# ZechengLi19/CIM

Measured on NVIDIA B200. Metric: CIM-head images/s (ROIAlign fwd+bwd + mask IoU + scoring fwd+bwd + mining + losses incl. PCL), higher is better.
Workload: dtype f32

## Files before the change

cim_b200/csrc/common.cuh:

```cuda
#pragma once
#include <cuda_runtime.h>
#include <cuda_fp16.h>
#include <stdint.h>
#include "../../include/cimhead.h"

#if defined(__CUDA_ARCH__) && (__CUDA_ARCH__ < 1000)
#error "libcimhead is written for sm_100a (B200) only"
#endif

#define CIM_API extern "C" __attribute__((visibility("default")))

static inline int cim_launch_status() {
    cudaError_t e = cudaGetLastError();
    return e == cudaSuccess ? CIM_OK : (int)e;
}
static inline bool cim_aligned(const void *p, size_t a) { return ((uintptr_t)p % a) == 0; }
static inline int cim_num_sms() {
    int dev = 0, n = 148;
    if (cudaGetDevice(&dev) == cudaSuccess)
        cudaDeviceGetAttribute(&n, cudaDevAttrMultiProcessorCount, dev);
    return n > 0 ? n : 148;
}
static inline int cim_max_smem_optin() {
    int dev = 0, n = 0;
    if (cudaGetDevice(&dev) == cudaSuccess)
        cudaDeviceGetAttribute(&n, cudaDevAttrMaxSharedMemoryPerBlockOptin, dev);
    return n;
}

__device__ __forceinline__ uint32_t smem_u32(const void *p) {
    return (uint32_t)__cvta_generic_to_shared(p);
}
__device__ __forceinline__ void mbar_init(uint64_t *bar, uint32_t count) {
    asm volatile("mbarrier.init.shared::cta.b64 [%0], %1;" ::"r"(smem_u32(bar)), "r"(count));
}
__device__ __forceinline__ void mbar_expect_tx(uint64_t *bar, uint32_t bytes) {
    asm volatile("mbarrier.arrive.expect_tx.shared::cta.b64 _, [%0], %1;" ::"r"(smem_u32(bar)),
                 "r"(bytes)
                 : "memory");
}
__device__ __forceinline__ void mbar_wait(uint64_t *bar, uint32_t parity) {
    asm volatile(
        "{\n\t.reg .pred p;\n\t"
        "WAIT_%=:\n\t"
        "mbarrier.try_wait.parity.shared::cta.b64 p, [%0], %1, %2;\n\t"
        "@p bra DONE_%=;\n\t"
        "bra WAIT_%=;\n\t"
        "DONE_%=:\n\t}" ::"r"(smem_u32(bar)),
        "r"(parity), "r"(100000u)
        : "memory");
}
__device__ __forceinline__ bool elect_one() {
    uint32_t leader;
    asm volatile("{\n\t.reg .pred p;\n\telect.sync _|p, 0xffffffff;\n\tselp.u32 %0, 1, 0, p;\n\t}" : "=r"(leader));
    return leader != 0;
}
__device__ __forceinline__ void fence_mbar_init() {
    asm volatile("fence.mbarrier_init.release.cluster;" ::: "memory");
}
__device__ __forceinline__ void fence_proxy_async_smem() {
    asm volatile("fence.proxy.async.shared::cta;" ::: "memory");
}
__device__ __forceinline__ void bulk_g2s(void *smem_dst, const void *gmem_src, uint32_t bytes,
                                         uint64_t *bar) {
    asm volatile(
        "cp.async.bulk.shared::cluster.global.mbarrier::complete_tx::bytes [%0], [%1], %2, [%3];" ::
            "r"(smem_u32(smem_dst)),
        "l"(gmem_src), "r"(bytes), "r"(smem_u32(bar))
        : "memory");
}
__device__ __forceinline__ void bulk_s2g(void *gmem_dst, const void *smem_src, uint32_t bytes) {
    asm volatile("cp.async.bulk.global.shared::cta.bulk_group [%0], [%1], %2;" ::"l"(gmem_dst),
                 "r"(smem_u32(smem_src)), "r"(bytes)
                 : "memory");
}
__device__ __forceinline__ void bulk_commit() { asm volatile("cp.async.bulk.commit_group;" ::: "memory"); }
template <int N>
__device__ __forceinline__ void bulk_wait_read() {
    asm volatile("cp.async.bulk.wait_group.read %0;" ::"n"(N) : "memory");
}
template <int N>
__device__ __forceinline__ void bulk_wait() {
    asm volatile("cp.async.bulk.wait_group %0;" ::"n"(N) : "memory");
}
```

cim_b200/csrc/mask_overlap.cu:

```cuda
#include "common.cuh"

bool cim_mask_overlap_tc_eligible(int n, long long words);
int cim_mask_overlap_tc_launch(const uint32_t *packed, const int32_t *area, const int32_t *perm,
                               const uint32_t *umap_a, const uint32_t *umap_b, int bw, unsigned long long *visited,
                               const int32_t *tile_order, int n_img, int n, long long words, int32_t *inter,
                               __half *iou, __half *asy, cudaStream_t st);

namespace {

__device__ __forceinline__ uint32_t nibble_of(uint32_t four_bytes) {
    uint32_t m = __vcmpne4(four_bytes, 0u) & 0x08040201u;
    return (m * 0x01010101u) >> 24;
}

__global__ void mask_pack_kernel(const uint8_t *__restrict__ masks, uint32_t *__restrict__ packed,
                                 long long n_masks, long long hw, long long words) {
    const long long total = n_masks * words;
    const bool vec = (hw % 16) == 0 && (((uintptr_t)masks) % 16) == 0;
    for (long long idx = blockIdx.x * (long long)blockDim.x + threadIdx.x; idx < total;
         idx += (long long)gridDim.x * blockDim.x) {
        const long long m = idx / words, w = idx - m * words;
        const long long p0 = w * 32;
        const uint8_t *src = masks + m * hw + p0;
        uint32_t bits = 0;
        if (vec && p0 + 32 <= hw) {
            const uint4 a = __ldg(reinterpret_cast<const uint4 *>(src));
            const uint4 b = __ldg(reinterpret_cast<const uint4 *>(src) + 1);
            bits = nibble_of(a.x) | (nibble_of(a.y) << 4) | (nibble_of(a.z) << 8) | (nibble_of(a.w) << 12) |
                   (nibble_of(b.x) << 16) | (nibble_of(b.y) << 20) | (nibble_of(b.z) << 24) |
                   (nibble_of(b.w) << 28);
        } else {
            for (int i = 0; i < 32; ++i)
                if (p0 + i < hw && src[i] != 0) bits |= 1u << i;
        }
        packed[idx] = bits;
    }
}

__device__ __forceinline__ uint32_t bits16_of(const uint4 a) {
    return nibble_of(a.x) | (nibble_of(a.y) << 4) | (nibble_of(a.z) << 8) | (nibble_of(a.w) << 12);
}
__global__ void mask_pack_tiled_kernel(const uint8_t *__restrict__ masks, uint32_t *__restrict__ packed,
                                       long long n_masks, int H, int W, long long words) {
    const long long total = n_masks * words;
    const long long used = (long long)H * W / 32;
    const int bpr = W >> 4;
    const bool vec = (((uintptr_t)masks) % 16) == 0;
    for (long long idx = blockIdx.x * (long long)blockDim.x + threadIdx.x; idx < total;
         idx += (long long)gridDim.x * blockDim.x) {
        const long long m = idx / words, w = idx - m * words;
        uint32_t bits = 0;
        if (w < used) {
            const int blk = (int)(w >> 2), wi = (int)(w & 3), by = blk / bpr, bx = blk - by * bpr;
            const uint8_t *src = masks + m * (long long)H * W + (long long)(8 * by + 2 * wi) * W + 16 * bx;
            if (vec) {
                bits = bits16_of(__ldg(reinterpret_cast<const uint4 *>(src))) |
                       (bits16_of(__ldg(reinterpret_cast<const uint4 *>(src + W))) << 16);
            } else {
                for (int i = 0; i < 16; ++i) {
// ... 212 lines not shown
#pragma unroll
    for (int o = 16; o > 0; o >>= 1) {
        s += __shfl_xor_sync(0xffffffffu, s, o);
        alo = min(alo, __shfl_xor_sync(0xffffffffu, alo, o));
        ahi = max(ahi, __shfl_xor_sync(0xffffffffu, ahi, o));
        blo = min(blo, __shfl_xor_sync(0xffffffffu, blo, o));
        bhi = max(bhi, __shfl_xor_sync(0xffffffffu, bhi, o));
    }
    if (lane == 0) {
        area[m] = s;
        kinfo[m] = ahi >= 0 ? make_int4(1, alo + ahi, bhi >= 0 ? blo + bhi : 0, 0) : make_int4(0, 0, 0, 0);
    }
}

__global__ void __launch_bounds__(1024)
mask_sort_kernel(const int4 *__restrict__ kinfo_all, int n, int npad, int kb_per_row, int nkb,
                 int32_t *__restrict__ perm_all, int32_t *__restrict__ inv_all) {
    extern __shared__ __align__(16) unsigned char sort_smem[];
    int *key = reinterpret_cast<int *>(sort_smem);
    int *idx = key + npad;
    const int img = blockIdx.x, tid = threadIdx.x, nthr = blockDim.x;
    const int4 *ki = kinfo_all + (size_t)img * n;
    const int nby = kb_per_row > 0 ? (nkb + kb_per_row - 1) / kb_per_row : 0;
    for (int i = tid; i < npad; i += nthr) {
        int k = 0x7fffffff;
        if (i < n) {
            const int4 v = ki[i];
            if (!v.x) k = 0;
            else if (kb_per_row > 0) {
                const int st = min(2, (v.y * 3) / (2 * kb_per_row));
                k = (st << 24) | ((st & 1) ? (2 * nby - v.z) : v.z);
            } else k = v.y;
        }
        key[i] = k;
        idx[i] = i < n ? i : 0x7fffffff;
    }
    __syncthreads();
    for (int size = 2; size <= npad; size <<= 1)
        for (int stride = size >> 1; stride > 0; stride >>= 1) {
            for (int t = tid; t < (npad >> 1); t += nthr) {
                const int lo = 2 * t - (t & (stride - 1)), hi = lo + stride;
                const bool asc = (lo & size) == 0;
                const int ka = key[lo], kb = key[hi], ia = idx[lo], ib = idx[hi];
                const bool a_first = ka < kb || (ka == kb && ia < ib);
                if (asc ? !a_first : a_first) { key[lo] = kb; key[hi] = ka; idx[lo] = ib; idx[hi] = ia; }
            }
            __syncthreads();
        }
    int32_t *perm = perm_all + (size_t)img * n, *inv = inv_all + (size_t)img * n;
    for (int i = tid; i < n; i += nthr) { perm[i] = idx[i]; inv[idx[i]] = i; }
}

__global__ void __launch_bounds__(128)
mask_union_kernel(const uint32_t *__restrict__ kbmap_all, const int32_t *__restrict__ perm_all, int n, int bw,
                  uint32_t *__restrict__ umap_a, uint32_t *__restrict__ umap_b, int nrb, int ncb) {
    const int blk = blockIdx.x, img = blockIdx.y;
    const bool is_a = blk < nrb;
    const int bs = is_a ? 128 : 256, b0 = (is_a ? blk : blk - nrb) * bs, b1 = min(n, b0 + bs);
    const uint32_t *kbm = kbmap_all + (size_t)img * n * bw;
    const int32_t *perm = perm_all + (size_t)img * n;
    __shared__ int s_idx[256];
    for (int i = threadIdx.x; i < b1 - b0; i += blockDim.x) s_idx[i] = perm[b0 + i];
    __syncthreads();
    for (int j = threadIdx.x; j < bw; j += blockDim.x) {
        uint32_t u = 0;
#pragma unroll 8
        for (int i = 0; i < b1 - b0; ++i) u |= __ldg(kbm + (size_t)s_idx[i] * bw + j);
        if (is_a) umap_a[((size_t)img * nrb + blk) * bw + j] = u;
        else umap_b[((size_t)img * ncb + (blk - nrb)) * bw + j] = u;
    }
}

__global__ void __launch_bounds__(256)
mask_rank_kernel(const uint32_t *__restrict__ umap_a, const uint32_t *__restrict__ umap_b, int bw, int nrb, int ncb,
                 int per_img, int tpad, int32_t *__restrict__ tile_order) {
    extern __shared__ __align__(16) unsigned char sort_smem[];
    int *key = reinterpret_cast<int *>(sort_smem);
    int *idx = key + tpad;
    const int img = blockIdx.x, tid = threadIdx.x, nthr = blockDim.x;
    for (int t = tid; t < tpad; t += nthr) { key[t] = t < per_img ? 0 : 0x7fffffff; idx[t] = -1; }
    __syncthreads();
    for (int e = tid; e < per_img * bw; e += nthr) {
        const int t = e / bw, j = e - t * bw;
        int rem = t, ti = 0;
        while (rem >= ncb - (ti >> 1)) { rem -= ncb - (ti >> 1); ++ti; }
        const int tj = (ti >> 1) + rem;
        const int c = __popc(__ldg(umap_a + ((size_t)img * nrb + ti) * bw + j) &
                             __ldg(umap_b + ((size_t)img * ncb + tj) * bw + j));
        if (c) atomicSub(&key[t], c);
        if (j == 0) idx[t] = (img << 16) | (ti << 8) | tj;
    }
    __syncthreads();
    for (int size = 2; size <= tpad; size <<= 1)
        for (int stride = size >> 1; stride > 0; stride >>= 1) {
            for (int t = tid; t < (tpad >> 1); t += nthr) {
                const int lo = 2 * t - (t & (stride - 1)), hi = lo + stride;
                const bool asc = (lo & size) == 0;
                const int ka = key[lo], kb = key[hi], ia = idx[lo], ib = idx[hi];
                const bool a_first = ka < kb || (ka == kb && ia < ib);
                if (asc ? !a_first : a_first) { key[lo] = kb; key[hi] = ka; idx[lo] = ib; idx[hi] = ia; }
            }
            __syncthreads();
        }
    for (int t = tid; t < per_img; t += nthr) tile_order[(size_t)t * gridDim.x + img] = idx[t];
}

__global__ void __launch_bounds__(256)
mask_unpermute2_kernel(const __half *__restrict__ tmp_a, const __half *__restrict__ tmp_b,
                       const int32_t *__restrict__ inv_all, __half *__restrict__ out_a, __half *__restrict__ out_b,
                       int n) {
    extern __shared__ __align__(16) unsigned char unp_smem[];
    __half *ra = reinterpret_cast<__half *>(unp_smem), *rb = ra + n;
    const int i = blockIdx.x, img = blockIdx.y;
    const int32_t *inv = inv_all + (size_t)img * n;
    const size_t so = ((size_t)img * n + inv[i]) * n, d_o = ((size_t)img * n + i) * n;
    if ((n & 7) == 0) {
        const uint4 *sa = reinterpret_cast<const uint4 *>(tmp_a + so), *sb = reinterpret_cast<const uint4 *>(tmp_b + so);
        for (int j = threadIdx.x; j < n / 8; j += blockDim.x) {
            reinterpret_cast<uint4 *>(ra)[j] = __ldg(sa + j);
            reinterpret_cast<uint4 *>(rb)[j] = __ldg(sb + j);
        }
    } else {
        for (int j = threadIdx.x; j < n; j += blockDim.x) { ra[j] = tmp_a[so + j]; rb[j] = tmp_b[so + j]; }
    }
    __syncthreads();
    if ((n & 1) == 0) {
        for (int j = threadIdx.x; j < n / 2; j += blockDim.x) {
            const int c0 = inv[2 * j], c1 = inv[2 * j + 1];
            reinterpret_cast<__half2 *>(out_a + d_o)[j] = __halves2half2(ra[c0], ra[c1]);
            reinterpret_cast<__half2 *>(out_b + d_o)[j] = __halves2half2(rb[c0], rb[c1]);
        }
    } else {
        for (int j = threadIdx.x; j < n; j += blockDim.x) { out_a[d_o + j] = ra[inv[j]]; out_b[d_o + j] = rb[inv[j]]; }
    }
}

template <typename T>
__global__ void __launch_bounds__(256)
mask_unpermute_kernel(const T *__restrict__ tmp_all, const int32_t *__restrict__ inv_all, T *__restrict__ out_all,
                      int n) {
    extern __shared__ __align__(16) unsigned char unp_smem[];
// ... 93 lines not shown
    const long long total = n_masks * words;
    const int blocks = (int)min((long long)cim_num_sms() * 16, (total + 255) / 256);
    mask_pack_kernel<<<blocks, 256, 0, (cudaStream_t)stream>>>(masks, packed, n_masks, hw, words);
    return cim_launch_status();
}

CIM_API int cim_mask_pack_tiled(const uint8_t *masks, uint32_t *packed, int64_t n_masks, int H, int W, int64_t words,
                                cim_stream_t stream) {
    if (!masks || !packed || n_masks < 0 || H <= 0 || W <= 0 || words * 32 < (int64_t)H * W) return CIM_ERR_ARG;
    if ((H & 7) || (W & 15)) return CIM_ERR_SHAPE;
    if (n_masks == 0) return CIM_OK;
    const long long total = n_masks * words;
    const int blocks = (int)min((long long)cim_num_sms() * 16, (total + 255) / 256);
    mask_pack_tiled_kernel<<<blocks, 256, 0, (cudaStream_t)stream>>>(masks, packed, n_masks, H, W, words);
    return cim_launch_status();
}

CIM_API int cim_mask_unpack_crops_tiled(const uint32_t *crop_words, const int32_t *crop_meta, const int64_t *crop_off,
                                        uint32_t *packed, int64_t n_masks, int H, int W, int64_t words,
                                        cim_stream_t stream) {
    if (!crop_words || !crop_meta || !crop_off || !packed || n_masks < 0 || H <= 0 || W <= 0) return CIM_ERR_ARG;
    if (words * 32 < (int64_t)H * W) return CIM_ERR_ARG;
    if ((H & 7) || (W & 15)) return CIM_ERR_SHAPE;
    if (n_masks == 0) return CIM_OK;
    if (n_masks > 0x7fffffffLL) return CIM_ERR_SHAPE;
    cudaStream_t st = (cudaStream_t)stream;
    cudaMemsetAsync(packed, 0, sizeof(uint32_t) * (size_t)n_masks * words, st);
    mask_unpack_crops_tiled_kernel<<<(unsigned)n_masks, 128, 0, st>>>(crop_words, crop_meta,
                                                                      reinterpret_cast<const long long *>(crop_off),
                                                                      packed, H, W, words);
    return cim_launch_status();
}

CIM_API int cim_mask_unpack_crops(const uint32_t *crop_words, const int32_t *crop_meta, const int64_t *crop_off,
                                  uint32_t *packed, int64_t n_masks, int H, int W, int64_t words,
                                  cim_stream_t stream) {
    if (!crop_words || !crop_meta || !crop_off || !packed || n_masks < 0 || H <= 0 || W <= 0) return CIM_ERR_ARG;
    if (words * 32 < (int64_t)H * W) return CIM_ERR_ARG;
    if (n_masks == 0) return CIM_OK;
    if (n_masks > 0x7fffffffLL) return CIM_ERR_SHAPE;
    cudaStream_t st = (cudaStream_t)stream;
    cudaMemsetAsync(packed, 0, sizeof(uint32_t) * (size_t)n_masks * words, st);
    mask_unpack_crops_kernel<<<(unsigned)n_masks, 128, 0, st>>>(crop_words, crop_meta,
                                                                reinterpret_cast<const long long *>(crop_off), packed,
                                                                H, W, words);
    return cim_launch_status();
}

namespace {
struct OverlapWs {
    unsigned long long *visited;
    int32_t *area;
    int4 *kinfo;
    uint32_t *kbmap, *umap_a, *umap_b;
    int32_t *perm, *inv, *tmp_inter, *tile_order;
    __half *tmp_iou, *tmp_asy;
    int bw;
    size_t bytes;
};
inline size_t up256(size_t v) { return (v + 255) & ~(size_t)255; }
OverlapWs carve_overlap_ws(void *base, int n_img, int n, long long words, int want_inter) {
    OverlapWs w{};
    const size_t nm = (size_t)(n_img > 0 ? n_img : 0) * (size_t)(n > 0 ? n : 0), nn = nm * (size_t)(n > 0 ? n : 0);
    const size_t nrb = (size_t)n_img * ((n + 127) / 128), ncb = (size_t)n_img * ((n + 255) / 256);
    const long long nkb = (words + 3) / 4;
    w.bw = (int)((nkb + 31) / 32);
    char *p = (char *)base;
    size_t o = 0;
    auto take = [&](size_t bytes) { char *q = p ? p + o : nullptr; o += up256(bytes); return q; };
    w.visited = (unsigned long long *)take(8);
    w.area = (int32_t *)take(nm * 4);
    w.kinfo = (int4 *)take(nm * 16);
    w.kbmap = (uint32_t *)take(nm * w.bw * 4);
    w.perm = (int32_t *)take(nm * 4);
    w.inv = (int32_t *)take(nm * 4);
    w.umap_a = (uint32_t *)take(nrb * w.bw * 4);
    w.umap_b = (uint32_t *)take(ncb * w.bw * 4);
    w.tile_order = (int32_t *)take(nrb * ((size_t)(n + 255) / 256) * 4);
    w.tmp_iou = (__half *)take(nn * 2);
    w.tmp_asy = (__half *)take(nn * 2);
    w.tmp_inter = want_inter ? (int32_t *)take(nn * 4) : nullptr;
    w.bytes = o + 256;
    return w;
}
}

namespace {
struct MaskMeta {
    int32_t *area;
    int4 *kinfo;
    uint32_t *kbmap;
    size_t bytes;
};
MaskMeta carve_meta(void *base, int n_img, int n, long long words) {
    MaskMeta m{};
    const size_t nm = (size_t)(n_img > 0 ? n_img : 0) * (size_t)(n > 0 ? n : 0);
    const int bw = (int)(((words + 3) / 4 + 31) / 32);
    char *p = (char *)base;
    size_t o = 0;
    auto take = [&](size_t bytes) { char *q = p ? p + o : nullptr; o += up256(bytes); return q; };
    m.area = (int32_t *)take(nm * 4);
    m.kinfo = (int4 *)take(nm * 16);
    m.kbmap = (uint32_t *)take(nm * bw * 4);
    m.bytes = o;
    return m;
}
}

CIM_API size_t cim_mask_meta_bytes(int n_img, int n, int64_t words) { return carve_meta(nullptr, n_img, n, words).bytes; }

CIM_API int cim_mask_meta(const uint32_t *packed, int n_img, int n, int64_t words, int kb_per_row, void *meta,
                          size_t meta_bytes, cim_stream_t stream) {
    if (!packed || !meta || n_img < 0 || n < 0 || words <= 0 || kb_per_row < 0) return CIM_ERR_ARG;
    if ((words & 3) || !cim_aligned(packed, 16)) return CIM_ERR_ALIGN;
    if (meta_bytes < cim_mask_meta_bytes(n_img, n, words) || !cim_aligned(meta, 256)) return CIM_ERR_WORKSPACE;
    if (n_img == 0 || n == 0) return CIM_OK;
    const MaskMeta m = carve_meta(meta, n_img, n, words);
    const long long n_masks = (long long)n_img * n;
    const int bw = (int)(((words + 3) / 4 + 31) / 32);
    mask_area_kernel<<<(unsigned)((n_masks + 7) / 8), 256, 0, (cudaStream_t)stream>>>(packed, m.area, m.kbmap, m.kinfo,
                                                                                       n_masks, words, bw, kb_per_row);
    return cim_launch_status();
}

CIM_API int cim_mask_unpack_crops_tiled_meta(const uint32_t *crop_words, const int32_t *crop_meta, const int64_t *crop_off,
                                             uint32_t *packed, void *meta, size_t meta_bytes, int n_img, int n, int H,
                                             int W, int64_t words, cim_stream_t stream) {
    if (!crop_words || !crop_meta || !crop_off || !packed || !meta || n_img < 0 || n < 0 || H <= 0 || W <= 0)
        return CIM_ERR_ARG;
    if ((H & 7) || (W & 15)) return CIM_ERR_SHAPE;
    if (words * 32 != (int64_t)H * W || (words & 3) || !cim_aligned(packed, 16)) return CIM_ERR_ALIGN;
    if (meta_bytes < cim_mask_meta_bytes(n_img, n, words) || !cim_aligned(meta, 256)) return CIM_ERR_WORKSPACE;
    if (n_img == 0 || n == 0) return CIM_OK;
    const MaskMeta mm = carve_meta(meta, n_img, n, words);
// ... 47 lines not shown
CIM_API int cim_mask_overlap_ex(const uint32_t *packed, int n_img, int n, int64_t words, int kb_per_row,
                                int32_t *inter, int32_t *area, void *iou_f16, void *asy_f16, void *workspace,
                                size_t ws_bytes, int algo, cim_stream_t stream) {
    return cim_mask_overlap_meta(packed, nullptr, n_img, n, words, kb_per_row, inter, area, iou_f16, asy_f16, workspace,
                                 ws_bytes, algo, stream);
}

CIM_API int cim_mask_overlap_meta(const uint32_t *packed, const void *meta, int n_img, int n, int64_t words,
                                  int kb_per_row, int32_t *inter, int32_t *area, void *iou_f16, void *asy_f16,
                                  void *workspace, size_t ws_bytes, int algo, cim_stream_t stream) {
    if (algo != CIM_OVERLAP_AUTO && algo != CIM_OVERLAP_POPC && algo != CIM_OVERLAP_TENSOR) return CIM_ERR_ARG;
    if (!packed || !iou_f16 || !asy_f16 || n_img < 0 || n < 0 || words <= 0 || kb_per_row < 0) return CIM_ERR_ARG;
    if (words * 32 >= (1LL << 24)) return CIM_ERR_SHAPE;
    if (n_img == 0 || n == 0) return CIM_OK;
    if (n_img > 65535 || n > 16384) return CIM_ERR_SHAPE;
    cudaStream_t st = (cudaStream_t)stream;
    const bool tc_ok = cim_mask_overlap_tc_eligible(n, words) && cim_aligned(packed, 16);
    if (algo == CIM_OVERLAP_TENSOR && !tc_ok) return CIM_ERR_SHAPE;
    const bool use_tc = algo == CIM_OVERLAP_TENSOR || (algo == CIM_OVERLAP_AUTO && tc_ok && n >= 256 && words >= 128);
    const size_t need = use_tc ? cim_mask_overlap_workspace_bytes(n_img, n, words, inter != nullptr)
                               : (area ? 0 : 2 * up256(sizeof(int32_t) * (size_t)n_img * n) + 512);
    if (need && (!workspace || ws_bytes < need || !cim_aligned(workspace, 256))) return CIM_ERR_WORKSPACE;
    OverlapWs w = carve_overlap_ws(workspace, n_img, n, words, inter != nullptr);
    const long long n_masks = (long long)n_img * n;
    int rc;
    if (meta) {
        if (!cim_aligned(meta, 256) || (words & 3)) return CIM_ERR_ALIGN;
        const MaskMeta mm = carve_meta(const_cast<void *>(meta), n_img, n, words);
        if (area) cudaMemcpyAsync(area, mm.area, sizeof(int32_t) * (size_t)n_masks, cudaMemcpyDeviceToDevice, st);
        area = mm.area;
        w.kinfo = mm.kinfo;
        w.kbmap = mm.kbmap;
    } else {
        if (!area) area = w.area;
        mask_area_kernel<<<(unsigned)((n_masks + 7) / 8), 256, 0, st>>>(packed, area, use_tc ? w.kbmap : nullptr,
                                                                        use_tc ? w.kinfo : nullptr, n_masks, words, w.bw,
                                                                        kb_per_row);
        if ((rc = cim_launch_status())) return rc;
    }
    __half *iou = reinterpret_cast<__half *>(iou_f16), *asy = reinterpret_cast<__half *>(asy_f16);
    if (use_tc) {
        int npad = 1;
        while (npad < n) npad <<= 1;
        const int nrb = (n + 127) / 128, ncb = (n + 255) / 256;
        int per_img = 0;
        for (int i = 0; i < nrb; ++i) per_img += ncb - (i >> 1);
        int tpad = 1;
        while (tpad < per_img) tpad <<= 1;
        const bool ordered = n_img < 32768 && nrb < 256 && ncb < 256 && (size_t)tpad * 8 <= 48 * 1024;
        const size_t smem_sort = (size_t)npad * 8;
        cudaFuncSetAttribute(mask_sort_kernel, cudaFuncAttributeMaxDynamicSharedMemorySize, (int)smem_sort);
        mask_sort_kernel<<<n_img, 1024, smem_sort, st>>>(w.kinfo, n, npad, kb_per_row, (int)((words + 3) / 4), w.perm,
                                                         w.inv);
        mask_union_kernel<<<dim3((unsigned)(nrb + ncb), (unsigned)n_img), 128, 0, st>>>(w.kbmap, w.perm, n, w.bw,
                                                                                        w.umap_a, w.umap_b, nrb, ncb);
        if (ordered)
            mask_rank_kernel<<<n_img, 256, (size_t)tpad * 8, st>>>(w.umap_a, w.umap_b, w.bw, nrb, ncb, per_img, tpad,
                                                                    w.tile_order);
        if ((rc = cim_launch_status())) return rc;
        cudaMemsetAsync(w.visited, 0, 8, st);
        const int32_t *order = ordered ? w.tile_order : nullptr;
        rc = cim_mask_overlap_tc_launch(packed, area, w.perm, w.umap_a, w.umap_b, w.bw, w.visited, order, n_img, n,
                                        words, w.tmp_inter, w.tmp_iou, w.tmp_asy, st);
        if (rc) return rc;
        dim3 g((unsigned)n, (unsigned)n_img);
        if ((size_t)n * 4 > 48 * 1024)
            cudaFuncSetAttribute(mask_unpermute2_kernel, cudaFuncAttributeMaxDynamicSharedMemorySize, n * 4);
        mask_unpermute2_kernel<<<g, 256, (size_t)n * 4, st>>>(w.tmp_iou, w.tmp_asy, w.inv, iou, asy, n);
        if (inter) {
            cudaFuncSetAttribute(mask_unpermute_kernel<int32_t>, cudaFuncAttributeMaxDynamicSharedMemorySize, n * 4);
            mask_unpermute_kernel<int32_t><<<g, 256, (size_t)n * 4, st>>>(w.tmp_inter, w.inv, inter, n);
        }
        return cim_launch_status();
    }
    const int nt = (n + TS - 1) / TS;
    dim3 grid((unsigned)(nt * (nt + 1) / 2), (unsigned)n_img);
    mask_overlap_popc_kernel<<<grid, 256, 0, st>>>(packed, area, n, words, inter, iou, asy);
    return cim_launch_status();
}
```

cim_b200/csrc/mask_overlap_tc.cu:

```cuda
#include "common.cuh"

namespace {

constexpr int TM = 128, TN = 256;
constexpr int KB = 128;
constexpr int ROW_BYTES = KB / 2;
constexpr int A_COLS = ROW_BYTES / 4;
constexpr int TMEM_COLS = 512;
constexpr int TMEM_A0 = TN;
constexpr int TMEM_SF = 448, SF_COLS = 64;
constexpr int B_BYTES = TN * ROW_BYTES;
constexpr int NEXP = 24;
constexpr int NEPI = 16;
constexpr int MMA_WARP = NEXP;
constexpr int THREADS = (NEXP + 1) * 32;
constexpr int FULL_ARRIVALS = 4 + 8;
constexpr size_t SI_BYTES = (size_t)(TM + 2 * TN) * 4 + 3 * (size_t)TM * 130 * 2;

constexpr int KLIST = 16384;
constexpr int SLOT_BYTES = NEXP * 32 * 16;

template <int STAGES_, int PF_ = 4>
struct Cfg {
    static constexpr int STAGES = STAGES_;
// ... 31 lines not shown
        "setp.ne.b32 p, %4, 0;\n\t"
        "tcgen05.mma.cta_group::1.kind::mxf4.block_scale.block32 [%0], [%1], %2, %3, [%5], [%5], p;\n\t}" ::"r"(tmem_d),
        "r"(tmem_a), "l"(bdesc), "r"(IDESC), "r"(accumulate), "r"(tmem_sf)
        : "memory");
}
__device__ __forceinline__ void tc_st16(uint32_t taddr, const uint32_t (&v)[16]) {
    asm volatile(
        "tcgen05.st.sync.aligned.32x32b.x16.b32 [%0], "
        "{%1,%2,%3,%4,%5,%6,%7,%8,%9,%10,%11,%12,%13,%14,%15,%16};" ::"r"(taddr),
        "r"(v[0]), "r"(v[1]), "r"(v[2]), "r"(v[3]), "r"(v[4]), "r"(v[5]), "r"(v[6]), "r"(v[7]), "r"(v[8]), "r"(v[9]),
        "r"(v[10]), "r"(v[11]), "r"(v[12]), "r"(v[13]), "r"(v[14]), "r"(v[15])
        : "memory");
    asm volatile("tcgen05.wait::st.sync.aligned;" ::: "memory");
}
__device__ __forceinline__ void tc_ld32(uint32_t taddr, int (&v)[32]) {
    asm volatile(
        "tcgen05.ld.sync.aligned.32x32b.x32.b32 "
        "{%0,%1,%2,%3,%4,%5,%6,%7,%8,%9,%10,%11,%12,%13,%14,%15,%16,%17,%18,%19,%20,%21,%22,%23,%24,%25,%26,%27,"
        "%28,%29,%30,%31}, [%32];"
        : "=r"(v[0]), "=r"(v[1]), "=r"(v[2]), "=r"(v[3]), "=r"(v[4]), "=r"(v[5]), "=r"(v[6]), "=r"(v[7]), "=r"(v[8]),
          "=r"(v[9]), "=r"(v[10]), "=r"(v[11]), "=r"(v[12]), "=r"(v[13]), "=r"(v[14]), "=r"(v[15]), "=r"(v[16]),
          "=r"(v[17]), "=r"(v[18]), "=r"(v[19]), "=r"(v[20]), "=r"(v[21]), "=r"(v[22]), "=r"(v[23]), "=r"(v[24]),
          "=r"(v[25]), "=r"(v[26]), "=r"(v[27]), "=r"(v[28]), "=r"(v[29]), "=r"(v[30]), "=r"(v[31])
        : "r"(taddr)
        : "memory");
    asm volatile("tcgen05.wait::ld.sync.aligned;" ::: "memory");
}

__device__ __forceinline__ void expand32_a(uint32_t w, uint32_t *o) {
    o[0] = w & 0x11111111u; o[1] = w & 0x22222222u; o[2] = w & 0x44444444u; o[3] = (w >> 1) & 0x44444444u;
}
__device__ __forceinline__ void expand32_b(uint32_t w, uint32_t *o) {
    o[0] = (w << 2) & 0x44444444u; o[1] = w & 0x22222222u; o[2] = (w >> 2) & 0x11111111u; o[3] = (w >> 3) & 0x11111111u;
}
__device__ __forceinline__ void sts16(uint32_t saddr, uint32_t a, uint32_t b, uint32_t c, uint32_t d) {
    asm volatile("st.shared.v4.b32 [%0], {%1, %2, %3, %4};" ::"r"(saddr), "r"(a), "r"(b), "r"(c), "r"(d) : "memory");
}

__device__ __forceinline__ float rcp_approx(float x) {
    float r;
    asm("rcp.approx.ftz.f32 %0, %1;" : "=f"(r) : "f"(x));
    return r;
}
__device__ __forceinline__ __half ratio_f16(float fi, float fd, float rcp_d) {
    float q = fi * rcp_d;
    const int low = (int)(__float_as_uint(q) & 0x1FFFu) - 0x1000;
    const bool easy = (q == 0.f || q >= 6.2e-5f) && (low > 8 || low < -8);
    if (!easy) q = __fdiv_rn(fi, fd);
    return __float2half_rn(q);
}

template <class K>
__global__ void __launch_bounds__(THREADS, 1)
mask_overlap_tc_kernel(const uint32_t *__restrict__ packed, const int32_t *__restrict__ area_all,
                       const int32_t *__restrict__ perm_all, const uint32_t *__restrict__ umap_a,
                       const uint32_t *__restrict__ umap_b, int bw, unsigned long long *__restrict__ visited,
                       const int32_t *__restrict__ tile_order, int n, long long words, int n_img, int32_t *__restrict__ inter_all, __half *__restrict__ iou_all,
                       __half *__restrict__ asy_all) {
    constexpr int STAGES = K::STAGES;
    extern __shared__ unsigned char smem_raw[];
    unsigned char *smem = reinterpret_cast<unsigned char *>(((uintptr_t)smem_raw + 1023) & ~(uintptr_t)1023);
    unsigned char *stages = smem;
    uint16_t *klist = reinterpret_cast<uint16_t *>(stages + (size_t)STAGES * B_BYTES);
    unsigned char *slots = reinterpret_cast<unsigned char *>(klist + KLIST);
    uint64_t *full = reinterpret_cast<uint64_t *>(smem + K::BODY_BYTES);
    uint64_t *empty = full + STAGES;
    uint64_t *accum_full = empty + STAGES;
    uint32_t *tmem_slot = reinterpret_cast<uint32_t *>(accum_full + 1);

    const int tid = threadIdx.x, lane = tid & 31, warp = tid >> 5;
    const int ncb = (n + TN - 1) / TN, nrb = (n + TM - 1) / TM;
    int img, ti, tj;
    if (tile_order) {
        const int code = __ldg(tile_order + blockIdx.x);
        img = code >> 16; ti = (code >> 8) & 255; tj = code & 255;
    } else {
        int d = 0, rem = blockIdx.x;
        for (;;) {
            const int cnt = min(nrb, 2 * (ncb - d)) * n_img;
            if (rem < cnt) break;
            rem -= cnt;
            ++d;
        }
        const int per_img = min(nrb, 2 * (ncb - d));
        img = rem / per_img; ti = rem - img * per_img; tj = (ti >> 1) + d;
    }
    const int row0 = ti * TM, col0 = tj * TN;

    if (tid == 0) {
        for (int s = 0; s < STAGES; ++s) { mbar_init(&full[s], FULL_ARRIVALS); mbar_init(&empty[s], 1); }
        mbar_init(accum_full, 1);
        fence_mbar_init();
    }
    if (warp == MMA_WARP) {
        asm volatile("tcgen05.alloc.cta_group::1.sync.aligned.shared::cta.b32 [%0], %1;" ::"r"(smem_u32(tmem_slot)),
                     "r"((uint32_t)TMEM_COLS)
                     : "memory");
        asm volatile("tcgen05.relinquish_alloc_permit.cta_group::1.sync.aligned;" ::: "memory");
    }
    const int32_t *perm = perm_all + (size_t)img * n;
    const uint32_t *ua = umap_a + ((size_t)img * nrb + ti) * bw, *ub = umap_b + ((size_t)img * ncb + tj) * bw;
    int nkb = 0;
    for (int j = lane; j < bw; j += 32) nkb += __popc(__ldg(ua + j) & __ldg(ub + j));
#pragma unroll
    for (int o = 16; o > 0; o >>= 1) nkb += __shfl_xor_sync(0xffffffffu, nkb, o);
    if (tid == 0 && visited) atomicAdd(visited, (unsigned long long)nkb);

    for (int c = warp; c * 32 < bw; c += THREADS / 32) {
        int pre = 0;
        for (int j = lane; j < c * 32; j += 32) pre += __popc(__ldg(ua + j) & __ldg(ub + j));
#pragma unroll
        for (int o = 16; o > 0; o >>= 1) pre += __shfl_xor_sync(0xffffffffu, pre, o);
        const int j = c * 32 + lane;
        uint32_t mj = j < bw ? (__ldg(ua + j) & __ldg(ub + j)) : 0u;
        int incl = __popc(mj);
#pragma unroll
        for (int o = 1; o < 32; o <<= 1) {
            const int t = __shfl_up_sync(0xffffffffu, incl, o);
            if (lane >= o) incl += t;
        }
        int off = pre + incl - __popc(mj);
        while (mj) {
            const int b = __ffs(mj) - 1;
            mj &= mj - 1;
            if (off < KLIST) klist[off] = (uint16_t)(j * 32 + b);
            ++off;
        }
    }
    tc_fence_before();
    __syncthreads();
    tc_fence_after();
    const uint32_t tmem_base = *tmem_slot;
    if (warp < 4) {
        uint32_t one[16];
#pragma unroll
        for (int i = 0; i < 16; ++i) one[i] = 0x7F7F7F7Fu;
        for (int c = 0; c < SF_COLS; c += 16) tc_st16(tmem_base + ((uint32_t)(32 * warp) << 16) + TMEM_SF + c, one);
        tc_fence_before();
    }
    __syncthreads();
    tc_fence_after();
    if (warp < NEXP) {
        const bool is_a = warp < 8;
        const int grp = is_a ? (warp >> 2) : ((warp - 8) >> 3);
        const int r = is_a ? 32 * (warp & 3) + lane : 32 * ((warp - 8) & 7) + lane;
        const uint32_t a_lane = tmem_base + ((uint32_t)(32 * (warp & 3)) << 16) + TMEM_A0;
        uint32_t chunk[4];
#pragma unroll
        for (int c = 0; c < 4; ++c) chunk[c] = smem_u32(stages) + b_chunk_off(r, c);
        const int g = is_a ? row0 + r : col0 + r;
        const bool valid = g < n;
        const uint32_t *rp = packed + ((size_t)img * n + (size_t)(valid ? __ldg(perm + g) : 0)) * words;
        const int nj = (nkb - grp + 1) >> 1;
        constexpr int PF = K::PF;
        const uint32_t klist_s = smem_u32(klist);
        const uint32_t slot0 = smem_u32(slots) + (uint32_t)tid * 16u;
        auto process = [&](int j, const uint4 &p) {
            const int i = 2 * j + grp, u = i / STAGES, s = i - u * STAGES;
            uint32_t o[16];
            const uint32_t pw[4] = {p.x, p.y, p.z, p.w};
            if (is_a) {
#pragma unroll
                for (int q = 0; q < 4; ++q) expand32_a(pw[q], o + 4 * q);
            } else {
#pragma unroll
                for (int q = 0; q < 4; ++q) expand32_b(pw[q], o + 4 * q);
            }
            if (u > 0) mbar_wait(&empty[s], (u - 1) & 1);
            if (is_a) {
                tc_st16(a_lane + (uint32_t)(s * A_COLS), o);
                tc_fence_before();
            } else {
                const uint32_t so = (uint32_t)s * B_BYTES;
#pragma unroll
                for (int q = 0; q < 4; ++q) sts16(chunk[q] + so, o[4 * q], o[4 * q + 1], o[4 * q + 2], o[4 * q + 3]);
#ifndef CIM_OV_ABL_NOFENCE
                fence_proxy_async_smem();
#endif
            }
            __syncwarp();
            if (lane == 0) mbar_arrive(&full[s]);
        };
        auto fetch = [&](int j, int d) {
            if (j < nj) {
                uint32_t kbi;
                asm volatile("ld.shared.u16 %0, [%1];" : "=r"(kbi) : "r"(klist_s + (uint32_t)(2 * j + grp) * 2u) : "memory");
#ifndef CIM_OV_ABL_NOLOAD
                asm volatile("cp.async.cg.shared.global [%0], [%1], 16, %2;" ::"r"(slot0 + (uint32_t)d * SLOT_BYTES),
                             "l"(rp + (size_t)kbi * 4), "r"(valid ? 16u : 0u) : "memory");
#else
                if (kbi == 0xFFFFFu) asm volatile("cp.async.cg.shared.global [%0], [%1], 16, %2;" ::"r"(slot0 + (uint32_t)d * SLOT_BYTES),
                             "l"(rp + (size_t)kbi * 4), "r"(valid ? 16u : 0u) : "memory");
#endif
            }
            asm volatile("cp.async.commit_group;" ::: "memory");
        };
#pragma unroll
        for (int d = 0; d < PF; ++d) fetch(d, d);
        for (int j0 = 0; j0 < nj; j0 += PF) {
#pragma unroll
            for (int d = 0; d < PF; ++d) {
                const int j = j0 + d;
                if (j < nj) {
                    asm volatile("cp.async.wait_group %0;" ::"n"(PF - 1) : "memory");
                    uint4 p;
                    asm volatile("ld.shared.v4.u32 {%0, %1, %2, %3}, [%4];"
                                 : "=r"(p.x), "=r"(p.y), "=r"(p.z), "=r"(p.w) : "r"(slot0 + (uint32_t)d * SLOT_BYTES) : "memory");
                    process(j, p);
                    fetch(j + PF, d);
                }
            }
        }
        asm volatile("cp.async.wait_group 0;" ::: "memory");
    } else {
        if (elect_one() && nkb > 0) {
            const uint64_t bd0 = smem_desc(smem_u32(stages));
            const uint32_t a0 = tmem_base + TMEM_A0, sf = tmem_base + TMEM_SF;
            uint32_t ph = 0;
            for (int kb0 = 0; kb0 < nkb; kb0 += STAGES) {
#pragma unroll
                for (int s = 0; s < STAGES; ++s) {
                    const int kb = kb0 + s;
                    if (kb < nkb) {
                        mbar_wait(&full[s], ph);
                        tc_fence_after();
                        const uint64_t bd = bd0 + (uint64_t)(s * (B_BYTES >> 4));
                        const uint32_t a_t = a0 + (uint32_t)(s * A_COLS);
#ifndef CIM_OV_ABL_NOMMA
                        tc_mma_mxf4_ts(tmem_base, a_t, bd, sf, kb != 0);
#pragma unroll
                        for (int k = 1; k < KB / 64; ++k)
                            tc_mma_mxf4_ts(tmem_base, a_t + 8 * k, bd + 2 * k, sf, 1u);
#endif
                        tc_commit(&empty[s]);
                    }
                }
                ph ^= 1;
            }
            tc_commit(accum_full);
        }
        __syncwarp();
    }

    constexpr int EP = 130;
    int *areaR = reinterpret_cast<int *>(stages);
// ... 65 lines not shown
            for (int rr = warp; rr < TM; rr += NEPI) {
                const int gr = row0 + rr, gc = cpass + 4 * lane;
                if (gr >= n || gc >= n) continue;
                const uint32_t *pi = reinterpret_cast<const uint32_t *>(s_iou + rr * EP + 4 * lane);
                const uint32_t *pa = reinterpret_cast<const uint32_t *>(s_asy + rr * EP + 4 * lane);
                const size_t o = (size_t)gr * n + gc;
                if (vec_ok && gc + 4 <= n) {
                    *reinterpret_cast<uint2 *>(iou + o) = make_uint2(pi[0], pi[1]);
                    *reinterpret_cast<uint2 *>(asy + o) = make_uint2(pa[0], pa[1]);
                } else {
                    for (int e = 0; e < 4 && gc + e < n; ++e) {
                        iou[o + e] = s_iou[rr * EP + 4 * lane + e];
                        asy[o + e] = s_asy[rr * EP + 4 * lane + e];
                    }
                }
            }
            if (mirror) {
                for (int cc = warp; cc < 128; cc += NEPI) {
                    const int gc = cpass + cc;
                    if (gc >= n) break;
#pragma unroll
                    for (int h = 0; h < TM / 32; ++h) {
                        const int rr = h * 32 + lane, gr = row0 + rr;
                        if (gr >= n) continue;
                        const size_t o = (size_t)gc * n + gr;
                        iou[o] = s_iou[rr * EP + cc];
                        asy[o] = s_asyT[rr * EP + cc];
                    }
                }
            }
            asm volatile("bar.sync 1, %0;" ::"n"(NEPI * 32) : "memory");
        }
    }
#ifdef CIM_OV_ABL_NOEPI
epi_done:
#endif
    tc_fence_before();
    __syncthreads();
    if (warp == MMA_WARP) {
        tc_fence_after();
        asm volatile("tcgen05.dealloc.cta_group::1.sync.aligned.b32 %0, %1;" ::"r"(tmem_base), "r"((uint32_t)TMEM_COLS)
                     : "memory");
    }
}

#ifndef CIM_OV_STAGES
#define CIM_OV_STAGES 8
#endif
#ifndef CIM_OV_PF
#define CIM_OV_PF 4
#endif

template <class K>
static int launch(const uint32_t *packed, const int32_t *area, const int32_t *perm, const uint32_t *umap_a,
                  const uint32_t *umap_b, int bw, unsigned long long *visited, const int32_t *tile_order, int n_img,
                  int n, long long words, int32_t *inter, __half *iou, __half *asy, cudaStream_t st) {
    const int nrb = (n + TM - 1) / TM, ncb = (n + TN - 1) / TN;
    int tiles = 0;
    for (int i = 0; i < nrb; ++i) tiles += ncb - (i >> 1);
    cudaFuncSetAttribute(mask_overlap_tc_kernel<K>, cudaFuncAttributeMaxDynamicSharedMemorySize, (int)K::SMEM_BYTES);
    mask_overlap_tc_kernel<K><<<(unsigned)(tiles * n_img), THREADS, K::SMEM_BYTES, st>>>(
        packed, area, perm, umap_a, umap_b, bw, visited, tile_order, n, words, n_img, inter, iou, asy);
    return cim_launch_status();
}

}

using CfgRun = Cfg<CIM_OV_STAGES, CIM_OV_PF>;

bool cim_mask_overlap_tc_eligible(int n, long long words) {
    return n >= 64 && words >= 4 && (words % 4) == 0 && (words + 3) / 4 <= KLIST &&
           (size_t)cim_max_smem_optin() >= CfgRun::SMEM_BYTES;
}

int cim_mask_overlap_tc_launch(const uint32_t *packed, const int32_t *area, const int32_t *perm,
                               const uint32_t *umap_a, const uint32_t *umap_b, int bw, unsigned long long *visited,
                               const int32_t *tile_order, int n_img, int n, long long words, int32_t *inter,
                               __half *iou, __half *asy, cudaStream_t st) {
    return launch<CfgRun>(packed, area, perm, umap_a, umap_b, bw, visited, tile_order, n_img, n, words, inter, iou, asy, st);
}
```

Baseline: 2250.

## Pre-gather sparse mask operands into block-major layout for the overlap kernel

Adds a union kernel that, alongside the per-128-row block union bitmaps, writes a compacted block-major operand buffer holding only the non-empty 16-byte chunks of each sorted mask, interleaved across the block's 128 rows. The tensor-core overlap kernel then fetches coalesced 16B chunks from this buffer, and the column-side union map is derived by OR-ing two row-block unions instead of keeping a separate 256-row map. Per-chunk membership bits are packed into the klist entries so zero-fill is decided without a permutation lookup. This removes scattered per-row gathers through perm, at the cost of an extra gather/write pass and more workspace memory.

Result: no change. 2253, median of 6 (+0.1%).

```diff
diff --git a/cim_b200/csrc/common.cuh b/cim_b200/csrc/common.cuh
--- a/cim_b200/csrc/common.cuh
+++ b/cim_b200/csrc/common.cuh
@@ -55,6 +55,10 @@
     asm volatile("{\n\t.reg .pred p;\n\telect.sync _|p, 0xffffffff;\n\tselp.u32 %0, 1, 0, p;\n\t}" : "=r"(leader));
     return leader != 0;
 }
+__device__ __forceinline__ uint32_t cim_ub_word(const uint32_t *u, int bw, int nrb, int tj, int j) {
+    const uint32_t lo = __ldg(u + (size_t)(2 * tj) * bw + j);
+    return 2 * tj + 1 < nrb ? lo | __ldg(u + (size_t)(2 * tj + 1) * bw + j) : lo;
+}
 __device__ __forceinline__ void fence_mbar_init() {
     asm volatile("fence.mbarrier_init.release.cluster;" ::: "memory");
 }
diff --git a/cim_b200/csrc/mask_overlap.cu b/cim_b200/csrc/mask_overlap.cu
--- a/cim_b200/csrc/mask_overlap.cu
+++ b/cim_b200/csrc/mask_overlap.cu
@@ -1,10 +1,9 @@
 #include "common.cuh"
 
 bool cim_mask_overlap_tc_eligible(int n, long long words);
-int cim_mask_overlap_tc_launch(const uint32_t *packed, const int32_t *area, const int32_t *perm,
-                               const uint32_t *umap_a, const uint32_t *umap_b, int bw, unsigned long long *visited,
-                               const int32_t *tile_order, int n_img, int n, long long words, int32_t *inter,
-                               __half *iou, __half *asy, cudaStream_t st);
+int cim_mask_overlap_tc_launch(const uint4 *opnd, const int32_t *area, const int32_t *perm, const uint32_t *umap,
+                               int bw, unsigned long long *visited, const int32_t *tile_order, int n_img, int n,
+                               long long words, int32_t *inter, __half *iou, __half *asy, cudaStream_t st);
 
 namespace {
 
@@ -323,27 +322,37 @@
 }
 
 __global__ void __launch_bounds__(128)
-mask_union_kernel(const uint32_t *__restrict__ kbmap_all, const int32_t *__restrict__ perm_all, int n, int bw,
-                  uint32_t *__restrict__ umap_a, uint32_t *__restrict__ umap_b, int nrb, int ncb) {
-    const int blk = blockIdx.x, img = blockIdx.y;
-    const bool is_a = blk < nrb;
-    const int bs = is_a ? 128 : 256, b0 = (is_a ? blk : blk - nrb) * bs, b1 = min(n, b0 + bs);
-    const uint32_t *kbm = kbmap_all + (size_t)img * n * bw;
-    const int32_t *perm = perm_all + (size_t)img * n;
-    __shared__ int s_idx[256];
-    for (int i = threadIdx.x; i < b1 - b0; i += blockDim.x) s_idx[i] = perm[b0 + i];
+mask_union_opnd_kernel(const uint32_t *__restrict__ packed, const uint32_t *__restrict__ kbmap_all,
+                       const int32_t *__restrict__ perm_all, int n, long long words, int bw, int nrb,
+                       uint32_t *__restrict__ umap, uint4 *__restrict__ opnd) {
+    const int blk = blockIdx.x, j = blockIdx.y, img = blockIdx.z;
+    const int r = threadIdx.x, g = blk * 128 + r;
+    uint32_t m = 0;
+    const uint4 *row = nullptr;
+    if (g < n) {
+        const size_t mi = (size_t)img * n + __ldg(perm_all + (size_t)img * n + g);
+        m = __ldg(kbmap_all + mi * bw + j);
+        row = reinterpret_cast<const uint4 *>(packed + mi * words);
+    }
+    __shared__ uint32_t s_or[4];
+    const uint32_t wu = __reduce_or_sync(0xffffffffu, m);
+    if ((r & 31) == 0) s_or[r >> 5] = wu;
     __syncthreads();
-    for (int j = threadIdx.x; j < bw; j += blockDim.x) {
-        uint32_t u = 0;
-#pragma unroll 8
-        for (int i = 0; i < b1 - b0; ++i) u |= __ldg(kbm + (size_t)s_idx[i] * bw + j);
-        if (is_a) umap_a[((size_t)img * nrb + blk) * bw + j] = u;
-        else umap_b[((size_t)img * ncb + (blk - nrb)) * bw + j] = u;
+    uint32_t u = s_or[0] | s_or[1] | s_or[2] | s_or[3];
+    if (r == 0) umap[((size_t)img * nrb + blk) * bw + j] = u;
+    uint4 *dst = opnd + ((size_t)img * nrb + blk) * (size_t)(words >> 2) * 128 + r;
+    while (u) {
+        const int b = __ffs(u) - 1;
+        u &= u - 1;
+        const size_t kb = (size_t)j * 32 + b;
+        uint4 v = make_uint4(0u, 0u, 0u, 0u);
+        if ((m >> b) & 1u) v = __ldg(row + kb);
+        dst[kb * 128] = v;
     }
 }
 
 __global__ void __launch_bounds__(256)
-mask_rank_kernel(const uint32_t *__restrict__ umap_a, const uint32_t *__restrict__ umap_b, int bw, int nrb, int ncb,
+mask_rank_kernel(const uint32_t *__restrict__ umap, int bw, int nrb, int ncb,
                  int per_img, int tpad, int32_t *__restrict__ tile_order) {
     extern __shared__ __align__(16) unsigned char sort_smem[];
     int *key = reinterpret_cast<int *>(sort_smem);
@@ -356,8 +365,8 @@
         int rem = t, ti = 0;
         while (rem >= ncb - (ti >> 1)) { rem -= ncb - (ti >> 1); ++ti; }
         const int tj = (ti >> 1) + rem;
-        const int c = __popc(__ldg(umap_a + ((size_t)img * nrb + ti) * bw + j) &
-                             __ldg(umap_b + ((size_t)img * ncb + tj) * bw + j));
+        const uint32_t *u = umap + (size_t)img * nrb * bw;
+        const int c = __popc(__ldg(u + (size_t)ti * bw + j) & cim_ub_word(u, bw, nrb, tj, j));
         if (c) atomicSub(&key[t], c);
         if (j == 0) idx[t] = (img << 16) | (ti << 8) | tj;
     }
@@ -557,9 +566,10 @@
     unsigned long long *visited;
     int32_t *area;
     int4 *kinfo;
-    uint32_t *kbmap, *umap_a, *umap_b;
+    uint32_t *kbmap, *umap;
     int32_t *perm, *inv, *tmp_inter, *tile_order;
     __half *tmp_iou, *tmp_asy;
+    uint4 *opnd;
     int bw;
     size_t bytes;
 };
@@ -579,12 +589,12 @@
     w.kbmap = (uint32_t *)take(nm * w.bw * 4);
     w.perm = (int32_t *)take(nm * 4);
     w.inv = (int32_t *)take(nm * 4);
-    w.umap_a = (uint32_t *)take(nrb * w.bw * 4);
-    w.umap_b = (uint32_t *)take(ncb * w.bw * 4);
+    w.umap = (uint32_t *)take(nrb * w.bw * 4);
     w.tile_order = (int32_t *)take(nrb * ((size_t)(n + 255) / 256) * 4);
     w.tmp_iou = (__half *)take(nn * 2);
     w.tmp_asy = (__half *)take(nn * 2);
     w.tmp_inter = want_inter ? (int32_t *)take(nn * 4) : nullptr;
+    w.opnd = cim_mask_overlap_tc_eligible(n, words) ? (uint4 *)take(nrb * (size_t)nkb * 128 * 16) : nullptr;
     w.bytes = o + 256;
     return w;
 }
@@ -738,16 +748,15 @@
         cudaFuncSetAttribute(mask_sort_kernel, cudaFuncAttributeMaxDynamicSharedMemorySize, (int)smem_sort);
         mask_sort_kernel<<<n_img, 1024, smem_sort, st>>>(w.kinfo, n, npad, kb_per_row, (int)((words + 3) / 4), w.perm,
                                                          w.inv);
-        mask_union_kernel<<<dim3((unsigned)(nrb + ncb), (unsigned)n_img), 128, 0, st>>>(w.kbmap, w.perm, n, w.bw,
-                                                                                        w.umap_a, w.umap_b, nrb, ncb);
+        mask_union_opnd_kernel<<<dim3((unsigned)nrb, (unsigned)w.bw, (unsigned)n_img), 128, 0, st>>>(
+            packed, w.kbmap, w.perm, n, words, w.bw, nrb, w.umap, w.opnd);
         if (ordered)
-            mask_rank_kernel<<<n_img, 256, (size_t)tpad * 8, st>>>(w.umap_a, w.umap_b, w.bw, nrb, ncb, per_img, tpad,
-                                                                    w.tile_order);
+            mask_rank_kernel<<<n_img, 256, (size_t)tpad * 8, st>>>(w.umap, w.bw, nrb, ncb, per_img, tpad, w.tile_order);
         if ((rc = cim_launch_status())) return rc;
         cudaMemsetAsync(w.visited, 0, 8, st);
         const int32_t *order = ordered ? w.tile_order : nullptr;
-        rc = cim_mask_overlap_tc_launch(packed, area, w.perm, w.umap_a, w.umap_b, w.bw, w.visited, order, n_img, n,
-                                        words, w.tmp_inter, w.tmp_iou, w.tmp_asy, st);
+        rc = cim_mask_overlap_tc_launch(w.opnd, area, w.perm, w.umap, w.bw, w.visited, order, n_img, n, words,
+                                        w.tmp_inter, w.tmp_iou, w.tmp_asy, st);
         if (rc) return rc;
         dim3 g((unsigned)n, (unsigned)n_img);
         if ((size_t)n * 4 > 48 * 1024)
diff --git a/cim_b200/csrc/mask_overlap_tc.cu b/cim_b200/csrc/mask_overlap_tc.cu
--- a/cim_b200/csrc/mask_overlap_tc.cu
+++ b/cim_b200/csrc/mask_overlap_tc.cu
@@ -107,9 +107,9 @@
 
 template <class K>
 __global__ void __launch_bounds__(THREADS, 1)
-mask_overlap_tc_kernel(const uint32_t *__restrict__ packed, const int32_t *__restrict__ area_all,
-                       const int32_t *__restrict__ perm_all, const uint32_t *__restrict__ umap_a,
-                       const uint32_t *__restrict__ umap_b, int bw, unsigned long long *__restrict__ visited,
+mask_overlap_tc_kernel(const uint4 *__restrict__ opnd, const int32_t *__restrict__ area_all,
+                       const int32_t *__restrict__ perm_all, const uint32_t *__restrict__ umap, int bw,
+                       unsigned long long *__restrict__ visited,
                        const int32_t *__restrict__ tile_order, int n, long long words, int n_img, int32_t *__restrict__ inter_all, __half *__restrict__ iou_all,
                        __half *__restrict__ asy_all) {
     constexpr int STAGES = K::STAGES;
@@ -154,20 +154,23 @@
         asm volatile("tcgen05.relinquish_alloc_permit.cta_group::1.sync.aligned;" ::: "memory");
     }
     const int32_t *perm = perm_all + (size_t)img * n;
-    const uint32_t *ua = umap_a + ((size_t)img * nrb + ti) * bw, *ub = umap_b + ((size_t)img * ncb + tj) * bw;
+    const uint32_t *um = umap + (size_t)img * nrb * bw, *ua = um + (size_t)ti * bw;
     int nkb = 0;
-    for (int j = lane; j < bw; j += 32) nkb += __popc(__ldg(ua + j) & __ldg(ub + j));
+    for (int j = lane; j < bw; j += 32) nkb += __popc(__ldg(ua + j) & cim_ub_word(um, bw, nrb, tj, j));
 #pragma unroll
     for (int o = 16; o > 0; o >>= 1) nkb += __shfl_xor_sync(0xffffffffu, nkb, o);
     if (tid == 0 && visited) atomicAdd(visited, (unsigned long long)nkb);
 
+    const int bh0 = 2 * tj, bh1 = 2 * tj + 1 < nrb ? 2 * tj + 1 : -1;
     for (int c = warp; c * 32 < bw; c += THREADS / 32) {
         int pre = 0;
-        for (int j = lane; j < c * 32; j += 32) pre += __popc(__ldg(ua + j) & __ldg(ub + j));
+        for (int j = lane; j < c * 32; j += 32) pre += __popc(__ldg(ua + j) & cim_ub_word(um, bw, nrb, tj, j));
 #pragma unroll
         for (int o = 16; o > 0; o >>= 1) pre += __shfl_xor_sync(0xffffffffu, pre, o);
         const int j = c * 32 + lane;
-        uint32_t mj = j < bw ? (__ldg(ua + j) & __ldg(ub + j)) : 0u;
+        const uint32_t u0 = j < bw ? __ldg(um + (size_t)bh0 * bw + j) : 0u;
+        const uint32_t u1 = j < bw && bh1 >= 0 ? __ldg(um + (size_t)bh1 * bw + j) : 0u;
+        uint32_t mj = j < bw ? (__ldg(ua + j) & (u0 | u1)) : 0u;
         int incl = __popc(mj);
 #pragma unroll
         for (int o = 1; o < 32; o <<= 1) {
@@ -178,7 +181,7 @@
         while (mj) {
             const int b = __ffs(mj) - 1;
             mj &= mj - 1;
-            if (off < KLIST) klist[off] = (uint16_t)(j * 32 + b);
+            if (off < KLIST) klist[off] = (uint16_t)((j * 32 + b) | (((u0 >> b) & 1u) << 14) | (((u1 >> b) & 1u) << 15));
             ++off;
         }
     }
@@ -203,9 +206,9 @@
         uint32_t chunk[4];
 #pragma unroll
         for (int c = 0; c < 4; ++c) chunk[c] = smem_u32(stages) + b_chunk_off(r, c);
-        const int g = is_a ? row0 + r : col0 + r;
-        const bool valid = g < n;
-        const uint32_t *rp = packed + ((size_t)img * n + (size_t)(valid ? __ldg(perm + g) : 0)) * words;
+        const int blk = is_a ? ti : (bh1 >= 0 ? 2 * tj + (r >> 7) : bh0);
+        const int half_bit = is_a ? 14 : 14 + (r >> 7);
+        const uint4 *rp = opnd + ((size_t)img * nrb + blk) * (size_t)(words >> 2) * 128 + (r & 127);
         const int nj = (nkb - grp + 1) >> 1;
         constexpr int PF = K::PF;
         const uint32_t klist_s = smem_u32(klist);
@@ -238,14 +241,15 @@
         };
         auto fetch = [&](int j, int d) {
             if (j < nj) {
-                uint32_t kbi;
-                asm volatile("ld.shared.u16 %0, [%1];" : "=r"(kbi) : "r"(klist_s + (uint32_t)(2 * j + grp) * 2u) : "memory");
+                uint32_t e;
+                asm volatile("ld.shared.u16 %0, [%1];" : "=r"(e) : "r"(klist_s + (uint32_t)(2 * j + grp) * 2u) : "memory");
+                const uint32_t kbi = e & 0x3FFFu, bytes = (is_a || ((e >> half_bit) & 1u)) ? 16u : 0u;
 #ifndef CIM_OV_ABL_NOLOAD
                 asm volatile("cp.async.cg.shared.global [%0], [%1], 16, %2;" ::"r"(slot0 + (uint32_t)d * SLOT_BYTES),
-                             "l"(rp + (size_t)kbi * 4), "r"(valid ? 16u : 0u) : "memory");
+                             "l"(rp + (size_t)kbi * 128), "r"(bytes) : "memory");
 #else
                 if (kbi == 0xFFFFFu) asm volatile("cp.async.cg.shared.global [%0], [%1], 16, %2;" ::"r"(slot0 + (uint32_t)d * SLOT_BYTES),
-                             "l"(rp + (size_t)kbi * 4), "r"(valid ? 16u : 0u) : "memory");
+                             "l"(rp + (size_t)kbi * 128), "r"(bytes) : "memory");
 #endif
             }
             asm volatile("cp.async.commit_group;" ::: "memory");
@@ -417,15 +421,15 @@
 #endif
 
 template <class K>
-static int launch(const uint32_t *packed, const int32_t *area, const int32_t *perm, const uint32_t *umap_a,
-                  const uint32_t *umap_b, int bw, unsigned long long *visited, const int32_t *tile_order, int n_img,
-                  int n, long long words, int32_t *inter, __half *iou, __half *asy, cudaStream_t st) {
+static int launch(const uint4 *opnd, const int32_t *area, const int32_t *perm, const uint32_t *umap, int bw,
+                  unsigned long long *visited, const int32_t *tile_order, int n_img, int n, long long words,
+                  int32_t *inter, __half *iou, __half *asy, cudaStream_t st) {
     const int nrb = (n + TM - 1) / TM, ncb = (n + TN - 1) / TN;
     int tiles = 0;
     for (int i = 0; i < nrb; ++i) tiles += ncb - (i >> 1);
     cudaFuncSetAttribute(mask_overlap_tc_kernel<K>, cudaFuncAttributeMaxDynamicSharedMemorySize, (int)K::SMEM_BYTES);
     mask_overlap_tc_kernel<K><<<(unsigned)(tiles * n_img), THREADS, K::SMEM_BYTES, st>>>(
-        packed, area, perm, umap_a, umap_b, bw, visited, tile_order, n, words, n_img, inter, iou, asy);
+        opnd, area, perm, umap, bw, visited, tile_order, n, words, n_img, inter, iou, asy);
     return cim_launch_status();
 }
 
@@ -438,9 +442,8 @@
            (size_t)cim_max_smem_optin() >= CfgRun::SMEM_BYTES;
 }
 
-int cim_mask_overlap_tc_launch(const uint32_t *packed, const int32_t *area, const int32_t *perm,
-                               const uint32_t *umap_a, const uint32_t *umap_b, int bw, unsigned long long *visited,
-                               const int32_t *tile_order, int n_img, int n, long long words, int32_t *inter,
-                               __half *iou, __half *asy, cudaStream_t st) {
-    return launch<CfgRun>(packed, area, perm, umap_a, umap_b, bw, visited, tile_order, n_img, n, words, inter, iou, asy, st);
-}
+int cim_mask_overlap_tc_launch(const uint4 *opnd, const int32_t *area, const int32_t *perm, const uint32_t *umap,
+                               int bw, unsigned long long *visited, const int32_t *tile_order, int n_img, int n,
+                               long long words, int32_t *inter, __half *iou, __half *asy, cudaStream_t st) {
+    return launch<CfgRun>(opnd, area, perm, umap, bw, visited, tile_order, n_img, n, words, inter, iou, asy, st);
+}
```
